# jmhb0/view_neti

Hardware: AMD Instinct MI355X
Metric: TI train steps/sec (SD-1.5 512^2 bs=4 per GPU) (higher is better)
Workload: dtype f16; 1 GPU; learnable_mode 0, sd15 shapes, 512x512 fp16, bs=4/GPU, grad_accum 1, full train step (VAE+16xCLIP+UNet fwd/bwd+AdamW); global_batch=4, parallelism=dp1, rccl_ranks=1, hipgraph=True

## Files before the change

include/vneti.h:

```cpp
#ifndef VNETI_H
#define VNETI_H
#include <stddef.h>
#include <stdint.h>

#ifdef __cplusplus
extern "C" {
#endif

#define VNETI_ABI_VERSION 1

int vneti_version(void);
int vneti_precision(void);
int vneti_last_error(char* buf, size_t n);

typedef struct vneti_gemm_desc {
  const void* A;
  const void* B;
  void* C;
  long long lda, ldb, ldc;
  int M, N, K;
  int batch;
  long long strideA, strideB, strideC;
  const float* bias;
  const void* rowadd;
  long long ld_rowadd;
  int rows_per_group;
  const void* resid;
  long long ldr;
  float alpha;
  int act;
  int out_f32;
  int conv_mode;
  int Hi, Wi, Ci, Ho, Wo, stride, pad_t, pad_l, ups;
  long long ldx;
  int tile_hint;
  void* workspace;
  long long workspace_bytes;
  int split_k;
  const void* gate_src;
  long long ld_gate;
  int gate_act;
  void* C2;
  long long ldc2;
  int act2;
  void* gn_sums;
  int gn_hw, gn_cpg, gn_groups, gn_slots;
  int geglu;
  int conv_korder;
} vneti_gemm_desc;

int vneti_gemm_f16(const vneti_gemm_desc* d, void* stream);
int vneti_gemm_select_tile(int M, int N, int batch);
int vneti_gemm_select_split(int M, int N, int K, int batch, int tile_hint, long long workspace_bytes);

int vneti_im2col3x3_small(const void* x, int x_is_f32, long long sb, long long sc, long long sy,
                          long long sx, void* out, int Bn, int C, int Hi, int Wi, int Ho, int Wo,
                          int stride, int pad_t, int pad_l, void* stream);

int vneti_conv3x3_in(const void* x, int x_is_f32, long long sb, long long sc, long long sy, long long sx,
                     const void* w_packed, const float* bias, void* out, long long ldo, int Bn, int C, int H, int W,
                     int Co, void* gn_sums, int gn_groups, int gn_slots, void* stream);

int vneti_transpose_f16(const void* in, long long ld_in, long long stride_in, void* out,
                        long long ld_out, long long stride_out, int rows, int cols, int batch,
                        void* stream);
#define VNETI_TRANSPOSE_MAX 4
typedef struct vneti_transpose_desc {
  const void* inp;
  long long ld_in, stride_in;
  void* out;
  long long ld_out, stride_out;
  int rows, cols, batch, _pad;
} vneti_transpose_desc;
int vneti_transpose_f16_multi(const vneti_transpose_desc* descs, int n, void* stream);

long long vneti_groupnorm_ws_floats(int Bn, int HW, int C, int G);
int vneti_groupnorm_fwd(const void* x, long long ldx, void* y, long long ldy, const float* gamma,
                        const float* beta, float* mean, float* rstd, float* ws, int Bn, int HW,
                        int C, int G, float eps, int silu, void* stream);
int vneti_groupnorm_fwd_sums(const void* x, long long ldx, void* y, long long ldy, const float* gamma,
                             const float* beta, const void* sums, int slots, float* mean, float* rstd,
                             int Bn, int HW, int C, int G, float eps, int silu, void* stream);
int vneti_groupnorm_fwd_2l(const void* x, long long ldx, void* y, long long ldy, const float* gamma,
                           const float* beta, void* sums, int slots, float* mean, float* rstd, int Bn, int HW,
                           int C, int G, float eps, int silu, void* stream);
int vneti_groupnorm_bwd_2l(const void* dy, long long lddy, const void* x, long long ldx, const float* gamma,
                           const float* beta, const float* mean, const float* rstd, void* dx, long long lddx,
                           const void* dx_accum, long long ldacc, void* sums, int slots, float* ws, int Bn,
                           int HW, int C, int G, int silu, void* stream);
int vneti_groupnorm_bwd(const void* dy, long long lddy, const void* x, long long ldx,
                        const float* gamma, const float* beta, const float* mean,
                        const float* rstd, void* dx, long long lddx, const void* dx_accum,
                        long long ldacc, float* ws, int Bn, int HW, int C, int G, int silu,
                        void* stream);

int vneti_layernorm_fwd(const void* x, int x_is_f32, long long ldx, void* y, long long ldy,
                        const float* gamma, const float* beta, float* mean, float* rstd, int rows,
                        int C, float eps, void* stream);
int vneti_layernorm_bwd(const void* dy, int dy_is_f32, long long lddy, const void* x,
                        int x_is_f32, long long ldx, const float* gamma, const float* mean,
                        const float* rstd, void* dx, int dx_is_f32, long long lddx,
                        const void* dx_accum, long long ldacc, void* dx_f16_copy, long long ldcopy,
                        int rows, int C, void* stream);

int vneti_attn_fwd(const void* Q, long long ldq, const void* K, long long ldk, const void* V,
                   long long ldv, void* O, long long ldo, float* lse, int Bn, int H, int Nq,
// ... 156 lines not shown
```

view_neti_amd/csrc/gemm8.hip:

```cpp
#include <type_traits>

#include "common.h"
#include "gemm_args.h"

namespace {

constexpr int BM = 256, NT = 512;
constexpr int HALF_BYTES = 128 * 128;
constexpr int GN_IMG = 5;

#define VN_WAIT_VM(n) asm volatile("s_waitcnt vmcnt(" #n ")" ::: "memory")
#define VN_WAIT_LGKM0() asm volatile("s_waitcnt lgkmcnt(0)" ::: "memory")

template <int BN, int EPI, bool CONV, bool HALO = false>
__global__ __launch_bounds__(NT) void gemm8_kernel(GemmArgs g) {
  static_assert(BN == 256 || BN == 128, "tile width");
  static_assert(!HALO || (BN == 128 && CONV), "the halo-patch loop exists for the 256x128 convolution tile");
  constexpr int PATCH_STRIDE = 41 * 1024;
  constexpr bool H42 = HALO && BN == 128;
  constexpr int NJB = BN / 128;
  constexpr int HB_BYTES = (BN / 2) * 128;
  constexpr int HB_DMA = BN / 128;
  constexpr int NBUF = BN == 256 ? 2 : 3;
  constexpr int BUF_BYTES = 2 * HALF_BYTES + 2 * HB_BYTES;
  constexpr int CS_LD = BN + 8;
  constexpr int CS_BYTES = BM * CS_LD * 2;
  constexpr int LOOP_BYTES = HALO ? 2 * PATCH_STRIDE + 3 * 2 * HB_BYTES : NBUF * BUF_BYTES;
  constexpr int LDS_BYTES = CS_BYTES > LOOP_BYTES ? CS_BYTES : LOOP_BYTES;
  constexpr int GN_NG = BN / 4 + 2;
  const half_t* const e_gate = EPI == 2 ? g.gate_src : nullptr;
  half_t* const e_C2 = EPI == 2 ? g.C2 : nullptr;
  const int e_geglu = EPI == 2 ? g.geglu : 0;
  const int e_act = EPI == 2 ? g.act : 0;
  float* const e_gn_sums = EPI >= 1 ? g.gn_sums : nullptr;
  const half_t* const e_rowadd = EPI >= 1 ? g.rowadd : nullptr;
  const int e_conv = CONV ? g.conv_mode : 0;
  constexpr int GN_BYTES = EPI == 0 ? 0 : GN_IMG * GN_NG * 4 * 8;
  __shared__ __attribute__((aligned(16))) char smem[LDS_BYTES + GN_BYTES];

  const int tid = threadIdx.x;
  const int lane = tid & 63;
  const int wave = __builtin_amdgcn_readfirstlane(tid >> 6);
  const int wr = wave >> 2, wc = wave & 3;

  int nblk = g.tiles_m * g.tiles_n;
  int bid = blockIdx.x;
  {
    int q = nblk >> 3, r = nblk & 7, xcd = bid & 7, idx = bid >> 3;
    bid = (xcd < r ? xcd * (q + 1) : r * (q + 1) + (xcd - r) * q) + idx;
  }
  const int tile_m = bid / g.tiles_n;
  const int tile_n = bid - tile_m * g.tiles_n;
  const int m0 = tile_m * BM;
  const int n0 = tile_n * BN;
  const int bz = blockIdx.y;
  const int kz = blockIdx.z;
  int hb = 0, hty = 0, htx = 0, row0 = m0;
  if constexpr (HALO) {
    const int tpr = g.Wo >> 4, tpi = (g.Ho >> 4) * tpr;
    hb = tile_m / tpi;
    const int rem = tile_m - hb * tpi;
    hty = rem / tpr;
    htx = rem - hty * tpr;
    row0 = (hb * g.Ho + hty * 16) * g.Wo + htx * 16;
  }
  auto rowmem = [&](const int r) { return HALO ? row0 + (r >> 4) * g.Wo + (r & 15) : m0 + r; };

  const half_t* Ab = g.A + (long long)bz * g.strideA;
  const half_t* Bb = g.B + (long long)bz * g.strideB;
  const __amdgpu_buffer_rsrc_t rsA = vn_make_rsrc(Ab, g.a_bytes);
  const __amdgpu_buffer_rsrc_t rsB = vn_make_rsrc(Bb, g.b_bytes);

  const int lrow = tid >> 3;
  const int gchunk = (tid & 7) ^ ((lrow >> 1) & 7);
  const float rcp_hw = CONV ? 1.0f / (float)(g.Ho * g.Wo) : 0.f, rcp_wo = CONV ? 1.0f / (float)g.Wo : 0.f;
  int a_base[4];
  uint32_t a_mask[4];
#pragma unroll
  for (int r = 0; r < (HALO ? 0 : 4); ++r) {
    const int m = m0 + (r >> 1) * 128 + (r & 1) * 64 + lrow;
// ... 100 lines not shown
#pragma unroll
    for (int j = 0; j < 2; ++j)
      dma16(rsA, dst + j * 8192, nxt[j]);
  };
  auto issueB = [&](const int h, const int buf) {
    char* dst = smem + buf * BUF_BYTES + 2 * HALF_BYTES + h * HB_BYTES + wave * 1024;
    if constexpr (BN == 256) {
#pragma unroll
      for (int j = 0; j < 2; ++j) dma16(rsB, dst + j * 8192, nxt[j]);
    } else {
      dma16(rsB, dst, nxt[2 + h]);
    }
  };

  const int frow = lane & 15;
  const int fq = lane >> 4;
  const int fkey = (frow >> 1) & 7;
  int rdA[2], rdB[2];
#pragma unroll
  for (int s = 0; s < 2; ++s) {
    const int ch = ((s * 4 + fq) ^ fkey) << 4;
    rdA[s] = (wr * 64 + frow) * 128 + ch;
    rdB[s] = 2 * HALF_BYTES + (wc * (16 * NJB) + frow) * 128 + ch;
  }
  half8 af[4][2], bf0[NJB][2], bf1[NJB][2];
  auto readA = [&](const int h) {
#pragma unroll
    for (int i = 0; i < 4; ++i)
#pragma unroll
      for (int s = 0; s < 2; ++s)
        af[i][s] = as_half8(*reinterpret_cast<const u32x4*>(smem + rdA[s] + h * HALF_BYTES + i * 2048));
  };
  auto readB0 = [&](const int flip) {
#pragma unroll
    for (int jb = 0; jb < NJB; ++jb)
#pragma unroll
      for (int s = 0; s < 2; ++s)
        bf0[jb][s] = as_half8(*reinterpret_cast<const u32x4*>(smem + (rdB[s] ^ flip) + jb * 2048));
  };
  auto readB1 = [&]() {
#pragma unroll
    for (int jb = 0; jb < NJB; ++jb)
#pragma unroll
      for (int s = 0; s < 2; ++s)
        bf1[jb][s] = as_half8(*reinterpret_cast<const u32x4*>(smem + rdB[s] + HB_BYTES + jb * 2048));
  };

  const int wr4 = wave >> 1, wc2 = wave & 1;
  auto acc_row = [&](const int h, const int i) { return H42 ? wr4 * 64 + i * 16 + frow : h * 128 + wr * 64 + i * 16 + frow; };
  auto acc_col = [&](const int h, const int j, const int jb) {
    return H42 ? wc2 * 64 + (2 * h + j) * 16 + 4 * fq : j * (BN / 2) + wc * (16 * NJB) + jb * 16 + 4 * fq;
  };
  f32x4 bv[H42 ? 2 : 1][2][NJB];
  {
    const __amdgpu_buffer_rsrc_t rsBias = vn_make_rsrc(g.bias, g.bias ? (uint32_t)g.N * 4u : 0u);
#pragma unroll
    for (int h = 0; h < (H42 ? 2 : 1); ++h)
#pragma unroll
      for (int j = 0; j < 2; ++j)
#pragma unroll
        for (int jb = 0; jb < NJB; ++jb)
          bv[h][j][jb] = __builtin_bit_cast(f32x4, vn_buf_load16(rsBias, (uint32_t)(n0 + acc_col(h, j, jb)) * 4u));
  }
  f32x4 acc[2][2][4][NJB];
#pragma unroll
  for (int h = 0; h < 2; ++h)
#pragma unroll
    for (int j = 0; j < 2; ++j)
#pragma unroll
      for (int i = 0; i < 4; ++i)
#pragma unroll
        for (int jb = 0; jb < NJB; ++jb) acc[h][j][i][jb] = f32x4{0.f, 0.f, 0.f, 0.f};

#define VN_MMA(H, J, BF, PREP)                                                                                 \
  do {                                                                                                         \
    VN_WAIT_LGKM0();                                                                                           \
    __builtin_amdgcn_s_setprio(1);                                                                             \
    PREP;                                                                                                      \
    _Pragma("unroll") for (int s = 0; s < 2; ++s) _Pragma("unroll") for (int i = 0; i < 4; ++i)                \
        _Pragma("unroll") for (int jb = 0; jb < NJB; ++jb) acc[H][J][i][jb] =                                  \
            VN_MFMA_16x16x32(BF[jb][s], af[i][s], acc[H][J][i][jb], 0, 0, 0);                                  \
    __builtin_amdgcn_s_setprio(0);                                                                             \
  } while (0)
#define VN_PHASE_SYNC()                    \
  do {                                     \
    VN_WAIT_VM(10);                        \
    __builtin_amdgcn_s_barrier();          \
    __builtin_amdgcn_sched_barrier(0);     \
  } while (0)
#define VN_PHASE_END()                     \
  do {                                     \
    __builtin_amdgcn_s_barrier();          \
    __builtin_amdgcn_sched_barrier(0);     \
  } while (0)

#define VN_MMA2(H, PREP)                                                                                       \
  do {                                                                                                         \
    VN_WAIT_LGKM0();                                                                                           \
    __builtin_amdgcn_s_setprio(1);                                                                             \
    PREP;                                                                                                      \
    _Pragma("unroll") for (int s = 0; s < 2; ++s) _Pragma("unroll") for (int i = 0; i < 4; ++i) {              \
      acc[H][0][i][0] = VN_MFMA_16x16x32(bf0[0][s], af[i][s], acc[H][0][i][0], 0, 0, 0);                       \
      acc[H][1][i][0] = VN_MFMA_16x16x32(bf1[0][s], af[i][s], acc[H][1][i][0], 0, 0, 0);                       \
    }                                                                                                          \
    __builtin_amdgcn_s_setprio(0);                                                                             \
  } while (0)
#define VN_SYNC(n)                         \
  do {                                     \
    VN_WAIT_VM(n);                         \
    __builtin_amdgcn_s_barrier();          \
    __builtin_amdgcn_sched_barrier(0);     \
  } while (0)
  if constexpr (HALO) {
    constexpr int BRING = 2 * PATCH_STRIDE;
    auto patch_key = [](const int px) { return (int)((0x270745032ull >> (4 * (px >> 1))) & 7); };
    constexpr int PROW = 18 * 128;
    const int c_begin = kt_begin / 9, c_end = kt_end / 9;
    uint32_t pa_off[6];
#pragma unroll
    for (int j = 0; j < 6; ++j) {
      const int q = (j * 8 + wave) * 64 + lane, p = q >> 3, cs = q & 7;
      const int py = (p * 3641) >> 16;
      const int px = p - py * 18;
      const int iy = hty * 16 + py - 1, ix = htx * 16 + px - 1;
      const bool ok = p < 324 && (unsigned)iy < (unsigned)g.Hi && (unsigned)ix < (unsigned)g.Wi;
      pa_off[j] = ok ? (uint32_t)(((hb * g.Hi + iy) * g.Wi + ix) * g.ldx2 + ((cs ^ patch_key(px)) << 4)) : VN_OOB;
    }
    const int np_wave = wave == 0 ? 6 : 5;
    auto issueP = [&](const int j, const int chunk) {
      dma16(rsA, smem + (chunk & 1) * PATCH_STRIDE + (j * 8 + wave) * 1024, pa_off[j] + (uint32_t)chunk * 128u);
    };
    auto tap_dy = [&](const int tap) { const int dy = (tap * 11) >> 5; return e_conv == 2 ? 2 - dy : dy; };
    auto tap_dx = [&](const int tap) { const int dx = tap - 3 * ((tap * 11) >> 5); return e_conv == 2 ? 2 - dx : dx; };
    {
      constexpr int BBUF = 2 * HB_BYTES;
      auto issueBt = [&](const int kt, const int buf) {
        const uint32_t soff = (uint32_t)(kt_begin + kt) * 128u, dead = kt < T ? 0u : VN_OOB;
        char* dst = smem + BRING + buf * BBUF + wave * 1024;
        dma16(rsB, dst, (b_base[0] + soff) | dead);
        dma16(rsB, dst + HB_BYTES, (b_base[2] + soff) | dead);
      };
      int lb[3];
#pragma unroll
      for (int dx = 0; dx < 3; ++dx) lb[dx] = (wr4 * 4) * PROW + (frow + dx) * 128 + ((fq ^ patch_key(frow + dx)) << 4);
      const int rb0 = (wc2 * 64 + frow) * 128 + ((fq ^ fkey) << 4);
      half8 bfh[4][2];
      auto readAh = [&](const int half, const int ab) {
#pragma unroll
        for (int i = 2 * half; i < 2 * half + 2; ++i) {
          af[i][0] = as_half8(*reinterpret_cast<const u32x4*>(smem + ab + i * PROW));
          af[i][1] = as_half8(*reinterpret_cast<const u32x4*>(smem + (ab ^ 64) + i * PROW));
        }
      };
#define VN_MMA4(HALF, PREP)                                                                                    \
  do {                                                                                                         \
    VN_WAIT_LGKM0();                                                                                           \
    __builtin_amdgcn_s_setprio(1);                                                                             \
    PREP;                                                                                                      \
    _Pragma("unroll") for (int s = 0; s < 2; ++s) _Pragma("unroll") for (int i = 2 * HALF; i < 2 * HALF + 2; ++i) \
        _Pragma("unroll") for (int cb = 0; cb < 4; ++cb) {                                                     \
      acc[cb >> 1][cb & 1][i][0] =                                                                             \
          VN_MFMA_16x16x32(bfh[cb][s], af[i][s], acc[cb >> 1][cb & 1][i][0], 0, 0, 0);                         \
    }                                                                                                          \
    __builtin_amdgcn_s_setprio(0);                                                                             \
  } while (0)
      int abt[9];
#pragma unroll
      for (int k = 0; k < 9; ++k) {
        const int tp = e_conv == 2 ? 8 - k : k, dy = tp / 3, dx = tp - 3 * dy;
        abt[k] = (dx == 0 ? lb[0] : (dx == 1 ? lb[1] : lb[2])) + dy * PROW + (c_begin & 1) * PATCH_STRIDE;
      }
      uint32_t bo0 = b_base[0] + (uint32_t)(kt_begin + 2) * 128u, bo1 = b_base[2] + (uint32_t)(kt_begin + 2) * 128u;
      uint32_t pp[6];
#pragma unroll
      for (int j = 0; j < 6; ++j) pp[j] = pa_off[j] + (uint32_t)(c_begin + 1) * 128u;
      const bool w0 = wave == 0;
      char* const bring = smem + BRING + wave * 1024;
      auto readBh = [&](const int slot) {
        const char* b = smem + BRING + slot * BBUF;
#pragma unroll
        for (int cb = 0; cb < 4; ++cb) {
          bfh[cb][0] = as_half8(*reinterpret_cast<const u32x4*>(b + cb * 2048 + rb0));
          bfh[cb][1] = as_half8(*reinterpret_cast<const u32x4*>(b + cb * 2048 + (rb0 ^ 64)));
        }
      };
#pragma unroll
      for (int j = 0; j < 6; ++j)
// ... 112 lines not shown
      cur ^= 1;
#pragma unroll
      for (int s = 0; s < 2; ++s) {
        rdA[s] ^= BUF_BYTES;
        rdB[s] ^= BUF_BYTES;
      }
    }
  } else {
#pragma unroll
    for (int t0 = 0; t0 < 2; ++t0) {
      prepA(0);
      prepB(0);
      prepB(1);
      issueA(0, t0);
      issueB(0, t0);
      issueB(1, t0);
      prepA(1);
      issueA(1, t0);
    }
    prepA(0);
    prepB(0);
    prepB(1);
    VN_WAIT_VM(8);
    __builtin_amdgcn_s_barrier();
    __builtin_amdgcn_sched_barrier(0);
    if (wr == 1) __builtin_amdgcn_s_barrier();
    __builtin_amdgcn_sched_barrier(0);
    int stg = 2;
    for (int t = 0; t < T; ++t) {
      readB0(0);
      readB1();
      readA(0);
      issueA(0, stg);
      issueB(0, stg);
      issueB(1, stg);
      VN_SYNC(10);
      VN_MMA2(0, prepA(1));
      VN_PHASE_END();
      readA(1);
      issueA(1, stg);
      VN_SYNC(8);
      VN_MMA2(1, (prepA(0), prepB(0), prepB(1)));
      VN_PHASE_END();
      stg = stg == 2 ? 0 : stg + 1;
#pragma unroll
      for (int s = 0; s < 2; ++s) {
        rdA[s] = rdA[s] >= 2 * BUF_BYTES ? rdA[s] - 2 * BUF_BYTES : rdA[s] + BUF_BYTES;
        rdB[s] = rdB[s] >= 2 * BUF_BYTES ? rdB[s] - 2 * BUF_BYTES : rdB[s] + BUF_BYTES;
      }
    }
#undef VN_MMA2
#undef VN_SYNC
  }
  if (wr == 0) __builtin_amdgcn_s_barrier();
  asm volatile("s_waitcnt vmcnt(0) lgkmcnt(0)" ::: "memory");
  __syncthreads();
#undef VN_MMA
#undef VN_PHASE_SYNC
#undef VN_PHASE_END

  if (g.ksplit > 1) {
    float* ws = g.ws + ((long long)(kz * g.batch + bz) * g.M) * g.N;
    const __amdgpu_buffer_rsrc_t rsW = vn_make_rsrc(ws, 0x7fffffffu);
#pragma unroll
    for (int h = 0; h < 2; ++h)
#pragma unroll
      for (int j = 0; j < 2; ++j)
#pragma unroll
        for (int i = 0; i < 4; ++i)
#pragma unroll
          for (int jb = 0; jb < NJB; ++jb) {
            const int m = rowmem(acc_row(h, i));
            const int n = n0 + acc_col(h, j, jb);
            if (m < g.M && n < g.N) {
              float* p = ws + (long long)m * g.N + n;
              if (n + 4 <= g.N && (g.N & 3) == 0) {
                vn_st16_wt(rsW, (uint32_t)(((long long)m * g.N + n) * 4), acc[h][j][i][jb]);
              } else {
                for (int e = 0; e < 4 && n + e < g.N; ++e) p[e] = acc[h][j][i][jb][e];
              }
            }
          }
    return;
  }

  if (e_gn_sums && !(HALO && g.gn_hw == g.Ho * g.Wo)) {
    vn_u64* gacc = reinterpret_cast<vn_u64*>(smem + LDS_BYTES);
    for (int i = tid; i < GN_IMG * GN_NG * 4; i += NT) gacc[i] = 0;
  }
  {
    const int nsw = ((frow >> 3) & 1) << 2;
#pragma unroll
    for (int h = 0; h < 2; ++h)
#pragma unroll
      for (int i = 0; i < 4; ++i)
#pragma unroll
        for (int j = 0; j < 2; ++j)
#pragma unroll
          for (int jb = 0; jb < NJB; ++jb) {
            const int ml = acc_row(h, i);
            const int nl = acc_col(h, j, jb) ^ nsw;
            half4 o;
#pragma unroll
            for (int e = 0; e < 4; ++e)
              o[e] = (half_t)apply_act(acc[h][j][i][jb][e] * g.alpha + bv[H42 ? h : 0][j][jb][e], e_act);
            *reinterpret_cast<half4*>(smem + ((size_t)ml * CS_LD + nl) * 2) = o;
          }
  }
  __syncthreads();

  half_t* Cb = reinterpret_cast<half_t*>(g.C) + (long long)bz * g.strideC;
  const __amdgpu_buffer_rsrc_t rsC = vn_make_rsrc(Cb, 0x7fffffffu);
  const __amdgpu_buffer_rsrc_t rsC2 = vn_make_rsrc(e_C2, e_C2 ? 0x7fffffffu : 0u);
  const half_t* Rb = reinterpret_cast<const half_t*>(g.resid);
  if (Rb) Rb += (long long)bz * g.strideC;
  constexpr int CPR = BN / 8;
  constexpr int U = EPI == 2 ? 2 : (EPI == 1 ? 4 : (BN == 256 ? 8 : 4));
  static_assert(NT % CPR == 0 && CPR <= 32 && (BM * CPR) % NT == 0, "a thread keeps one 8-column chunk over all its rows");
  vn_u64* gacc = reinterpret_cast<vn_u64*>(smem + LDS_BYTES);
  const bool gn = e_gn_sums != nullptr;
  const float rcp_gnhw = gn ? 1.0f / (float)g.gn_hw : 0.f, rcp_rpg = e_rowadd ? 1.0f / (float)g.rows_per_group : 0.f;
  const int gn_img0 = gn ? row0 / g.gn_hw : 0, gn_g0t = gn ? n0 / g.gn_cpg : 0;
  const int c = (tid % CPR) * 8;
  const int n = n0 + c;
  const int gn_glo = gn ? n / g.gn_cpg : 0;
  const int gn_split = gn ? (gn_glo + 1) * g.gn_cpg - n : 8;
  int gn_img = -1;
  float s_lo = 0.f, q_lo = 0.f, s_hi = 0.f, q_hi = 0.f;
  auto gn_flush = [&]() {
    const int iref = __builtin_amdgcn_readfirstlane(gn_img);
    const bool uni = __all(gn_img == iref) && iref >= 0;
    if (uni) {
#pragma unroll
      for (int off = 32; off >= CPR; off >>= 1) {
        s_lo += __shfl_xor(s_lo, off);
        q_lo += __shfl_xor(q_lo, off);
        s_hi += __shfl_xor(s_hi, off);
        q_hi += __shfl_xor(q_hi, off);
      }
    }
    if (gn_img >= 0 && (!uni || lane < CPR)) {
      vn_u64* a = gacc + ((gn_img - gn_img0) * GN_NG + (gn_glo - gn_g0t)) * 4;
      vn_fx_add2(a, s_lo, q_lo);
      if (gn_split < 8) vn_fx_add2(a + 4, s_hi, q_hi);
    }
    s_lo = q_lo = s_hi = q_hi = 0.f;
  };
  const bool full_chunk = n + 8 <= g.N;
  const bool swap_halves = ((tid / CPR) >> 3) & 1;
  const __amdgpu_buffer_rsrc_t rsR = vn_make_rsrc(Rb, Rb ? 0x7fffffffu : 0u);
  const __amdgpu_buffer_rsrc_t rsRA = vn_make_rsrc(e_rowadd, e_rowadd ? 0x7fffffffu : 0u);
  const __amdgpu_buffer_rsrc_t rsG = vn_make_rsrc(e_gate, e_gate ? 0x7fffffffu : 0u);
  const int r_first = tid / CPR;
  constexpr int RPP = NT / CPR;
  const bool gn_one = HALO && gn && g.gn_hw == g.Ho * g.Wo;
  const bool ra_one = HALO && EPI >= 1 && e_rowadd && g.rows_per_group == g.Ho * g.Wo;
  half8 av_tile = half8{0, 0, 0, 0, 0, 0, 0, 0};
  if (ra_one) av_tile = as_half8(vn_buf_load16(rsRA, full_chunk ? (uint32_t)(((long long)hb * g.ld_rowadd + n) * 2) : VN_OOB));
  if (gn_one) gn_img = hb;
  for (int it0 = 0; it0 < BM / RPP; it0 += U) {
    half8 cv[U], rv[U], av[U], gv[U], gv2[U];
#pragma unroll
    for (int u = 0; u < U; ++u) {
      const int r = r_first + RPP * (it0 + u);
      const int m = rowmem(r);
      const bool ok = m < g.M && full_chunk;
      u32x4 t = *reinterpret_cast<const u32x4*>(smem + ((size_t)r * CS_LD + c) * 2);
      if (swap_halves) t = u32x4{t[2], t[3], t[0], t[1]};
      cv[u] = as_half8(t);
      if (Rb) rv[u] = as_half8(vn_buf_load16(rsR, ok ? (uint32_t)(((long long)m * g.ldr + n) * 2) : VN_OOB));
      if (EPI >= 1) {
        if (ra_one) {
          av[u] = av_tile;
        } else if (e_rowadd) {
          int grp = (int)((float)m * rcp_rpg);
          const int rem = m - grp * g.rows_per_group;
          grp += rem >= g.rows_per_group ? 1 : (rem < 0 ? -1 : 0);
          av[u] = as_half8(vn_buf_load16(rsRA, ok ? (uint32_t)(((long long)grp * g.ld_rowadd + n) * 2) : VN_OOB));
        }
      }
      if (EPI == 2 && e_gate) {
        const long long go = (long long)m * g.ld_gate + (e_geglu == 2 ? 2 * n : n);
        gv[u] = as_half8(vn_buf_load16_once(rsG, ok ? (uint32_t)(go * 2) : VN_OOB));
        gv2[u] = as_half8(vn_buf_load16_once(rsG, (ok && e_geglu == 2) ? (uint32_t)(go * 2 + 16) : VN_OOB));
// ... 10 lines not shown
          img = (int)((float)m * rcp_gnhw);
          const int rem = m - img * g.gn_hw;
          img += rem >= g.gn_hw ? 1 : (rem < 0 ? -1 : 0);
        }
        if (__any(img != gn_img)) {
          gn_flush();
          gn_img = img;
        }
      }
      if (!valid) continue;
      half8 v = cv[u];
      if (full_chunk) {
        if (EPI >= 1 && e_rowadd) {
          v = vn_add8(v, av[u]);
        }
        if (Rb) {
          v = vn_add8(v, rv[u]);
        }
        if (e_geglu == 2) {
#pragma unroll
          for (int c2 = 0; c2 < 2; ++c2) {
            const half8 pre = c2 == 0 ? gv[u] : gv2[u];
            half8 o;
#pragma unroll
            for (int e = 0; e < 4; ++e) {
              const float d = (float)v[4 * c2 + e], hh = (float)pre[e], gg = (float)pre[4 + e];
              float cdf, xpdf;
              vn_gelu_parts(gg, cdf, xpdf);
              o[e] = (half_t)(d * gg * cdf);
              o[4 + e] = (half_t)(d * hh * (cdf + xpdf));
            }
            vn_st16_wt(rsC, (uint32_t)(((long long)m * g.ldc + 2 * n + 8 * c2) * 2), o);
          }
          continue;
        }
        if (e_gate) {
#pragma unroll
          for (int e = 0; e < 8; ++e) v[e] = (half_t)((float)v[e] * act_grad((float)gv[u][e], g.gate_act));
        }
        if (e_geglu == 1 || (e_C2 && e_geglu == 0)) vn_st16_wt_saved(rsC, (uint32_t)(((long long)m * g.ldc + n) * 2), v);
        else vn_st16_wt(rsC, (uint32_t)(((long long)m * g.ldc + n) * 2), v);
        if (e_geglu == 1) {
          half4 o2;
#pragma unroll
          for (int e = 0; e < 4; ++e) o2[e] = (half_t)((float)v[e] * vn_gelu_erf((float)v[4 + e]));
          *reinterpret_cast<half4*>(e_C2 + (long long)m * g.ldc2 + (n >> 1)) = o2;
        }
        if (gn) {
          {
            const half2v one2 = {(half_t)1.f, (half_t)1.f};
#pragma unroll
            for (int e = 0; e < 8; e += 2) {
              const half2v p2 = {v[e], v[e + 1]};
              if (e < gn_split) {
                s_lo = VN_FDOT2(p2, one2, s_lo);
                q_lo = VN_FDOT2(p2, p2, q_lo);
              } else {
                s_hi = VN_FDOT2(p2, one2, s_hi);
                q_hi = VN_FDOT2(p2, p2, q_hi);
              }
            }
          }
        }
        if (e_C2 && e_geglu == 0) {
          half8 o2;
#pragma unroll
          for (int e = 0; e < 8; ++e) o2[e] = (half_t)apply_act((float)v[e], g.act2);
          vn_st16_wt(rsC2, (uint32_t)(((long long)m * g.ldc2 + n) * 2), o2);
        }
      } else {
        const half_t* radd = e_rowadd ? e_rowadd + (long long)(m / g.rows_per_group) * g.ld_rowadd + n : nullptr;
        for (int e = 0; e < 8 && n + e < g.N; ++e) {
          float x = (float)v[e];
          if (radd) x = (float)(half_t)(x + (float)radd[e]);
          if (Rb) x = (float)(half_t)(x + (float)Rb[(long long)m * g.ldr + n + e]);
          if (e_gate) x = (float)(half_t)(x * act_grad((float)e_gate[(long long)m * g.ld_gate + n + e], g.gate_act));
          Cb[(long long)m * g.ldc + n + e] = (half_t)x;
          if (e_C2) e_C2[(long long)m * g.ldc2 + n + e] = (half_t)apply_act((float)(half_t)x, g.act2);
          if (gn) {
            const float xs = (float)(half_t)x;
            if (e < gn_split) {
              s_lo += xs;
              q_lo += xs * xs;
            } else {
              s_hi += xs;
              q_hi += xs * xs;
            }
          }
        }
      }
    }
  }
  if (gn_one) {
    float v4[4] = {s_lo, q_lo, s_hi, q_hi};
#pragma unroll
    for (int k = 0; k < 4; ++k) {
      v4[k] += __shfl_xor(v4[k], 32);
      v4[k] += __shfl_xor(v4[k], 16);
    }
    static_assert(CPR == 16 || !HALO, "the halo tile is 128 columns wide");
    float* tab = reinterpret_cast<float*>(smem + LDS_BYTES);
    if (lane < 16) *reinterpret_cast<f32x4*>(tab + (wave * 16 + lane) * 4) = f32x4{v4[0], v4[1], v4[2], v4[3]};
    __syncthreads();
    if (tid < 32) {
      const int col = tid >> 1, half = tid & 1;
      float sv = 0.f, qv = 0.f;
#pragma unroll
      for (int w8 = 0; w8 < 8; ++w8) {
        sv += tab[(w8 * 16 + col) * 4 + 2 * half];
        qv += tab[(w8 * 16 + col) * 4 + 2 * half + 1];
      }
      const int nc = n0 + col * 8;
      const int glo = nc / g.gn_cpg;
      const int split = (glo + 1) * g.gn_cpg - nc;
      if (nc < g.N && (half == 0 || split < 8)) {
        const int slot = tile_m % g.gn_slots;
        vn_u64* dst = reinterpret_cast<vn_u64*>(e_gn_sums) + (((long long)hb * g.gn_slots + slot) * g.gn_G + glo + half) * 4;
        vn_fx_add2(dst, sv, qv);
      }
    }
  } else if (gn) {
    gn_flush();
    __syncthreads();
    const int slot = tile_m % g.gn_slots;
    for (int i = tid; i < GN_IMG * GN_NG; i += NT) {
      const vn_u64* src = gacc + 4 * i;
      if ((src[0] | src[1] | src[2] | src[3]) == 0) continue;
      const int img = gn_img0 + i / GN_NG, grp = gn_g0t + i % GN_NG;
      vn_u64* dst = reinterpret_cast<vn_u64*>(e_gn_sums) + (((long long)img * g.gn_slots + slot) * g.gn_G + grp) * 4;
#pragma unroll
      for (int w = 0; w < 4; ++w) atomicAdd(dst + w, src[w]);
    }
  }
}

inline int epilogue_level8(const GemmArgs& g) {
  if (g.gate_src || g.C2 || g.geglu || g.act) return 2;
  return (g.gn_sums || g.rowadd) ? 1 : 0;
}

}

int vneti_launch_gemm8(void* gemm_args, int bn, int halo, hipStream_t st) {
  GemmArgs& g = *reinterpret_cast<GemmArgs*>(gemm_args);
  if (g.out_f32 || (g.conv_mode && (g.ups || (g.conv_mode == 2 && g.stride == 2))) ||
      (g.M >= (1 << 24) && (g.conv_mode || g.rowadd || g.gn_sums)))
    return VNETI_EUNSUP;
  if (halo && (bn != 128 || g.conv_mode < 1 || g.conv_mode > 2 || g.stride != 1 || g.pad_t != 1 || g.pad_l != 1 || g.Hi != g.Ho ||
               g.Wi != g.Wo || (g.Ho & 15) || (g.Wo & 15) || (g.Ci & 63) || g.K != 9 * g.Ci || !g.korder ||
               g.batch != 1 || g.M != (g.M / (g.Ho * g.Wo)) * g.Ho * g.Wo))
    return VNETI_EUNSUP;
  if (halo && g.ksplit > 1) {
    const int nchunk = g.Ci / 64, cps = cdiv(nchunk, g.ksplit);
    g.kt_per_split = 9 * cps;
    g.ksplit = cdiv(nchunk, cps);
  }
  g.tiles_m = cdiv(g.M, BM);
  g.tiles_n = cdiv(g.N, bn);
  const dim3 grid(g.tiles_m * g.tiles_n, g.batch, g.ksplit), block(NT);
  const int epi = epilogue_level8(g);
#define VN_GO(E, C)                                                                        \
  do {                                                                                     \
    if (bn == 256) hipLaunchKernelGGL((gemm8_kernel<256, E, C>), grid, block, 0, st, g);   \
    else hipLaunchKernelGGL((gemm8_kernel<128, E, C>), grid, block, 0, st, g);             \
  } while (0)
#define VN_GO_HALO(E) hipLaunchKernelGGL((gemm8_kernel<128, E, true, true>), grid, block, 0, st, g)
  if (halo) {
    if (epi == 2) VN_GO_HALO(2); else if (epi == 1) VN_GO_HALO(1); else VN_GO_HALO(0);
  } else if (g.conv_mode) {
    if (epi == 2) VN_GO(2, true); else if (epi == 1) VN_GO(1, true); else VN_GO(0, true);
  } else {
    if (epi == 2) VN_GO(2, false); else if (epi == 1) VN_GO(1, false); else VN_GO(0, false);
  }
#undef VN_GO
#undef VN_GO_HALO
  return vneti_check_launch("gemm8_kernel");
}
```

view_neti_amd/lib.py:

```python
from __future__ import annotations

import ctypes as C
import keyword
import os
import re

_HERE = os.path.dirname(os.path.abspath(__file__))
HEADER_PATH = os.path.join(os.path.dirname(_HERE), "include", "vneti.h")

_PRECISIONS = {"fp16": ("libvneti_hip.so", 0), "bf16": ("libvneti_hip_bf16.so", 1)}
_precision = os.environ.get("VNETI_PRECISION", "fp16")
if _precision not in _PRECISIONS:
    raise RuntimeError(f"VNETI_PRECISION={_precision!r}: expected one of {sorted(_PRECISIONS)}")

_lib = None


def so_path(precision: str = None) -> str:
    return os.environ.get("VNETI_LIB_PATH") or os.path.join(_HERE, "csrc", _PRECISIONS[precision or _precision][0])


SO_PATH = so_path()


# ... 27 lines not shown
        return _SCALARS[base]
    if stars == 1 and base == "char":
        return C.c_char_p
    if stars == 1 and base in structs:
        return C.POINTER(structs[base])
    if stars and (base in _SCALARS or base in ("void", "char")):
        return C.c_void_p
    raise ValueError(f"vneti.h {where}: no ctypes rule for the type {ctype.strip()!r}")


def _declarator(decl: str, where: str):
    m = re.fullmatch(r"(.*[\s*])(\w+)", decl.strip(), re.S)
    if not m:
        raise ValueError(f"vneti.h {where}: cannot read the declaration {' '.join(decl.split())!r}")
    return m.group(1), m.group(2)


def parse_header(text: str):
    blank = lambda m: "\n" * m.group().count("\n")
    text = re.sub(r"/\*.*?\*/|//[^\n]*", blank, text, flags=re.S)
    text = re.sub(r'^[ \t]*#.*$|extern\s+"C"\s*\{|^\}[ \t]*$', "", text, flags=re.M)
    at = lambda src, pos: f"line {src.count(chr(10), 0, pos) + 1}"
    structs, protos = {}, {}
    typedef = r"typedef\s+struct\s+\w*\s*\{(.*?)\}\s*(\w+)\s*;"
    for m in re.finditer(typedef, text, flags=re.S):
        fields = []
        for d in re.finditer(r"[^;\s][^;]*", m.group(1)):
            where = at(text, m.start(1) + d.start())
            first, *more = d.group().split(",")
            ctype, name = _declarator(first, where)
            for n in [name] + [x.strip() for x in more]:
                if not n.isidentifier() or keyword.iskeyword(n):
                    raise ValueError(f"vneti.h {where}: cannot bind the field {n!r}")
                fields.append((n, _ctype(ctype, structs, where)))
        structs[m.group(2)] = type(m.group(2), (C.Structure,), {"_fields_": fields})
    rest = re.sub(typedef, blank, text, flags=re.S)
    for m in re.finditer(r"[^;\s][^;]*", rest):
        p = re.fullmatch(r"(int|long long)\s+(vneti_\w+)\s*\((.*)\)\s*", m.group(), re.S)
        if not p:
            raise ValueError(f"vneti.h {at(rest, m.start())}: cannot read {' '.join(m.group().split())!r} as a prototype")
        argtypes = []
        for x in re.finditer(r"[^,\s][^,]*", "" if p.group(3).strip() == "void" else p.group(3)):
            where = at(rest, m.start() + p.start(3) + x.start())
            argtypes.append(_ctype(_declarator(x.group(), where)[0], structs, where))
        protos[p.group(2)] = (_SCALARS[p.group(1)], argtypes)
    return structs, protos


with open(HEADER_PATH) as _f:
    _STRUCTS, _PROTOS = parse_header(_f.read())
GemmDesc, TransposeDesc = _STRUCTS["vneti_gemm_desc"], _STRUCTS["vneti_transpose_desc"]
SIGNATURES = {n[len("vneti_"):]: argtypes for n, (_, argtypes) in _PROTOS.items()}
VALUE_FUNCS = frozenset({
    "version", "precision", "last_error", "gemm_select_tile", "gemm_select_split", "img_resample_ksize",
    "groupnorm_ws_floats", "lpips_ws_floats", "mapper_num_params", "mapper_save_floats", "mapper_rowgrad_floats",
    "mapper_legacy_input_params"})
_stray = ({n[len("vneti_"):] for n, (res, _) in _PROTOS.items() if res is C.c_longlong} - VALUE_FUNCS) | (VALUE_FUNCS - set(SIGNATURES))
if _stray:
    raise RuntimeError(f"lib.VALUE_FUNCS is out of step with include/vneti.h: {sorted(_stray)}")


def declared_symbols() -> list[str]:
    src = open(HEADER_PATH).read()
    src = re.sub(r"/\*.*?\*/", "", src, flags=re.S)
    return sorted(set(re.findall(r"\b(vneti_[a-z0-9_]+)\s*\(", src)))


def load():
    global _lib
    if _lib is not None:
        return _lib
    if not os.path.exists(SO_PATH):
        raise RuntimeError(
            f"{os.path.basename(SO_PATH)} not found at {SO_PATH}: build it with "
            "`python view_neti_amd/csrc/build.py` (hipcc, gfx950). There is no fallback path.")
    lib = C.CDLL(SO_PATH)
    for name, (restype, argtypes) in _PROTOS.items():
        fn = getattr(lib, name, None)
        if fn is None:
            raise RuntimeError(f"{SO_PATH} does not export {name}, which include/vneti.h declares: rebuild it")
        fn.restype, fn.argtypes = restype, argtypes
    if lib.vneti_precision() != _PRECISIONS[_precision][1]:
        raise RuntimeError(f"{SO_PATH} computes in precision {lib.vneti_precision()}, the process asked for {_precision}")
    _lib = lib
    return lib


def last_error() -> str:
    lib = load()
    buf = C.create_string_buffer(512)
    lib.vneti_last_error(buf, 512)
    return buf.value.decode(errors="replace")


def check(rc: int, what: str = ""):
    if rc != 0:
        raise RuntimeError(f"vneti call failed ({what}) rc={rc}: {last_error()}")


def call(name: str, *args):
    check(getattr(load(), "vneti_" + name)(*args), name)


def query(name: str, *args) -> int:
    if name not in VALUE_FUNCS:
        raise KeyError(f"vneti_{name} returns a status: use call()")
    return int(getattr(load(), "vneti_" + name)(*args))
# ... 1 lines not shown
```

view_neti_amd/ops.py:

```python
from __future__ import annotations

import ctypes as C

import torch

from . import lib as _l

ACT_NONE, ACT_SILU, ACT_QUICK_GELU, ACT_GELU = 0, 1, 2, 3


def stream() -> int:
    return torch.cuda.current_stream().cuda_stream


def _p(t):
    return None if t is None else t.data_ptr()


def _ld(t):
    if t is None:
        return 0
    assert t.stride(-1) == 1, "last dim must be contiguous"
    return t.stride(-2) if t.dim() >= 2 else t.shape[-1]

# ... 337 lines not shown
def mapper_legacy_input_fwd(params_in, timesteps, w_pe, enc_out, nl, Bn, enc_dim, pe_dim, slot=None, slot_stride=0):
    _l.call("mapper_legacy_input_fwd", _p(params_in), _p(slot), slot_stride, _p(timesteps), _p(w_pe), _p(enc_out), nl, Bn,
            enc_dim, pe_dim, stream())


def mapper_legacy_input_fwd_slots(params_in, slots, slot_stride, timesteps, w_pe, enc_out, nl, Bn, enc_dim, pe_dim):
    _l.call("mapper_legacy_input_fwd_slots", _p(params_in), _p(slots), slot_stride, _p(timesteps), _p(w_pe), _p(enc_out),
            nl, Bn, enc_dim, pe_dim, stream())


def mapper_legacy_input_bwd(timesteps, w_pe, denc, grads_in, accumulate, nl, Bn, enc_dim, pe_dim, slot=None, slot_stride=0):
    _l.call("mapper_legacy_input_bwd", _p(timesteps), _p(w_pe), _p(denc), _p(grads_in), _p(slot), slot_stride,
            1 if accumulate else 0, nl, Bn, enc_dim, pe_dim, stream())


def text_embed(tok_emb, pos_emb, ids, pos_obj, word_obj, pos_view, word_view, X, nl, Bn, L, D):
    _l.call("text_embed", _p(tok_emb), _p(pos_emb), _p(ids), _p(pos_obj), _p(word_obj), _p(pos_view), _p(word_view),
            _p(X), nl, Bn, L, D, stream())


def text_final_fwd(last, gamma, beta, eps, pos_obj, byp_obj, alpha_obj, pos_view, byp_view, alpha_view, ctx_k, ctx_v,
                   nl, Bn, L, D, unconstrained_obj=False, unconstrained_view=False, norm_terms=None):
    _l.call("text_final_fwd", _p(last), _p(gamma), _p(beta), eps, _p(pos_obj), _p(byp_obj), alpha_obj,
            1 if unconstrained_obj else 0, _p(pos_view), _p(byp_view), alpha_view, 1 if unconstrained_view else 0,
            _p(norm_terms), _p(ctx_k), _p(ctx_v), nl, Bn, L, D, stream())


def text_final_bwd(last, gamma, eps, pos_obj, byp_obj, alpha_obj, dbyp_obj, pos_view, byp_view, alpha_view, dbyp_view,
                   dctx_k, dctx_v, dX, nl, Bn, L, D, unconstrained_obj=False, unconstrained_view=False,
                   norm_terms=None):
    _l.call("text_final_bwd", _p(last), _p(gamma), eps, _p(pos_obj), _p(byp_obj), alpha_obj,
            1 if unconstrained_obj else 0, _p(dbyp_obj), _p(pos_view), _p(byp_view), alpha_view,
            1 if unconstrained_view else 0, _p(dbyp_view), _p(norm_terms), _p(dctx_k), _p(dctx_v), _p(dX), nl, Bn, L,
            D, stream())


def cast_f32_f16(x, y):
    _l.call("cast_f32_f16", _p(x), _p(y), x.numel(), stream())


def mapper_inputs(timesteps, view_params, data, nl, Bn):
    nv = 0 if view_params is None else view_params.shape[1]
    _l.call("mapper_inputs", _p(timesteps), _p(view_params), nv, _p(data), nl, Bn, stream())


def gemm_select_split(M, N, K, batch, tile_hint, workspace_bytes):
    return _l.query("gemm_select_split", M, N, K, batch, tile_hint, workspace_bytes)


def gemm_select_tile(M, N, batch=1):
    return _l.query("gemm_select_tile", M, N, batch)


def lpips_prep(x, out, Bn, H, W):
    assert x.dtype == torch.float32 and x.shape == (Bn, 3, H, W)
    assert out.is_contiguous() and out.numel() >= Bn * H * W * 64
    _l.call("lpips_prep", _p(x), *x.stride(), _p(out), Bn, H, W, stream())


def relu_(x):
    assert x.is_contiguous()
    _l.call("relu_f16", _p(x), x.numel(), stream())


def relu_maxpool2x2(x, out, Bn, H, W, Cc):
    assert x.is_contiguous() and out.is_contiguous() and x.numel() >= Bn * H * W * Cc
    assert out.numel() >= Bn * (H // 2) * (W // 2) * Cc
    _l.call("relu_maxpool2x2_f16", _p(x), _p(out), Bn, H, W, Cc, stream())


def lpips_ws_floats(P, Cc, HW):
    n = _l.query("lpips_ws_floats", P, Cc, HW)
    if n < 0:
        raise RuntimeError(f"lpips_distance: unsupported shape P={P} C={Cc} HW={HW}")
    return n


def lpips_distance(feat, n_img, pairs, w, Cc, HW, ws, out, accumulate=False):
    P = pairs.shape[0]
    assert pairs.dtype == torch.int32 and pairs.is_contiguous() and pairs.shape == (P, 2)
    assert feat.is_contiguous() and feat.numel() >= n_img * HW * Cc and w.dtype == torch.float32 and w.numel() == Cc
    assert out.dtype == torch.float32 and out.numel() >= P and ws.dtype == torch.float32
    _l.call("lpips_distance", _p(feat), n_img, _p(pairs), P, _p(w), Cc, HW, _p(ws), ws.numel(), _p(out),
            1 if accumulate else 0, stream())


def img_resample_ksize(in_size, out_size, filt):
    return _l.query("img_resample_ksize", in_size, out_size, filt)


def img_resample_coeffs(in_size, out_size, filt, bounds, kk):
    _l.call("img_resample_coeffs", in_size, out_size, filt, _p(bounds), _p(kk), stream())


def img_resample_pass(inp, in_w, out, out_h, out_w, bounds, kk, ksize, horizontal):
    _l.call("img_resample_pass", _p(inp), in_w, _p(out), out_h, out_w, _p(bounds), _p(kk), ksize, 1 if horizontal else 0,
            stream())


def img_crop(inp, in_w, top, left, out, h, w, flip=False):
    _l.call("img_crop", _p(inp), in_w, top, left, _p(out), h, w, 1 if flip else 0, stream())


def img_enhance(img, h, w, mode, alpha, scratch8):
    _l.call("img_enhance", _p(img), h, w, mode, float(alpha), _p(scratch8), stream())

# ... 20 lines not shown
```

Measured before the change: 38.71 steps/s.

## Add 256-wide halo-patch convolution tile with wave-occupancy heuristic

Adds a 256x256 variant of the halo-patch implicit-GEMM convolution kernel. It has its own double-buffered B pipeline, a per-tap schedule, bias loading deferred until after the main loop, and a split GroupNorm partial-sum reduction through LDS. A heuristic picks it when N is a multiple of 256 and the estimated number of block waves favours wider tiles. The aim is more reuse of each loaded input patch across output channels and fewer passes over the activations. In exchange it uses more LDS and registers per block and gives fewer blocks per launch. An environment variable and API can force or disable the path.

After: 38.82 steps/s (median of 6 runs). No clear change (+0.3%).

```diff
diff --git a/include/vneti.h b/include/vneti.h
--- a/include/vneti.h
+++ b/include/vneti.h
@@ -52,6 +52,8 @@
 int vneti_gemm_f16(const vneti_gemm_desc* d, void* stream);
 int vneti_gemm_select_tile(int M, int N, int batch);
 int vneti_gemm_select_split(int M, int N, int K, int batch, int tile_hint, long long workspace_bytes);
+int vneti_gemm_halo_wide_set(int mode);
+int vneti_gemm_halo_wide_count(void);
 
 int vneti_im2col3x3_small(const void* x, int x_is_f32, long long sb, long long sc, long long sy,
                           long long sx, void* out, int Bn, int C, int Hi, int Wi, int Ho, int Wo,
diff --git a/view_neti_amd/csrc/gemm8.hip b/view_neti_amd/csrc/gemm8.hip
--- a/view_neti_amd/csrc/gemm8.hip
+++ b/view_neti_amd/csrc/gemm8.hip
@@ -1,3 +1,5 @@
+#include <atomic>
+#include <cstdlib>
 #include <type_traits>
 
 #include "common.h"
@@ -15,7 +17,7 @@
 template <int BN, int EPI, bool CONV, bool HALO = false>
 __global__ __launch_bounds__(NT) void gemm8_kernel(GemmArgs g) {
   static_assert(BN == 256 || BN == 128, "tile width");
-  static_assert(!HALO || (BN == 128 && CONV), "the halo-patch loop exists for the 256x128 convolution tile");
+  static_assert(!HALO || CONV, "the halo-patch loops are convolution tiles");
   constexpr int PATCH_STRIDE = 41 * 1024;
   constexpr bool H42 = HALO && BN == 128;
   constexpr int NJB = BN / 128;
@@ -25,7 +27,8 @@
   constexpr int BUF_BYTES = 2 * HALF_BYTES + 2 * HB_BYTES;
   constexpr int CS_LD = BN + 8;
   constexpr int CS_BYTES = BM * CS_LD * 2;
-  constexpr int LOOP_BYTES = HALO ? 2 * PATCH_STRIDE + 3 * 2 * HB_BYTES : NBUF * BUF_BYTES;
+  constexpr bool H44 = HALO && BN == 256;
+  constexpr int LOOP_BYTES = HALO ? 2 * PATCH_STRIDE + (H44 ? 2 : 3) * 2 * HB_BYTES : NBUF * BUF_BYTES;
   constexpr int LDS_BYTES = CS_BYTES > LOOP_BYTES ? CS_BYTES : LOOP_BYTES;
   constexpr int GN_NG = BN / 4 + 2;
   const half_t* const e_gate = EPI == 2 ? g.gate_src : nullptr;
@@ -232,7 +235,7 @@
     return H42 ? wc2 * 64 + (2 * h + j) * 16 + 4 * fq : j * (BN / 2) + wc * (16 * NJB) + jb * 16 + 4 * fq;
   };
   f32x4 bv[H42 ? 2 : 1][2][NJB];
-  {
+  auto load_bias = [&]() {
     const __amdgpu_buffer_rsrc_t rsBias = vn_make_rsrc(g.bias, g.bias ? (uint32_t)g.N * 4u : 0u);
 #pragma unroll
     for (int h = 0; h < (H42 ? 2 : 1); ++h)
@@ -241,7 +244,8 @@
 #pragma unroll
         for (int jb = 0; jb < NJB; ++jb)
           bv[h][j][jb] = __builtin_bit_cast(f32x4, vn_buf_load16(rsBias, (uint32_t)(n0 + acc_col(h, j, jb)) * 4u));
-  }
+  };
+  if constexpr (!H44) load_bias();
   f32x4 acc[2][2][4][NJB];
 #pragma unroll
   for (int h = 0; h < 2; ++h)
@@ -312,7 +316,137 @@
     };
     auto tap_dy = [&](const int tap) { const int dy = (tap * 11) >> 5; return e_conv == 2 ? 2 - dy : dy; };
     auto tap_dx = [&](const int tap) { const int dx = tap - 3 * ((tap * 11) >> 5); return e_conv == 2 ? 2 - dx : dx; };
-    {
+    if constexpr (H44) {
+      constexpr int BBUF = 2 * HB_BYTES;
+      int lb[3];
+#pragma unroll
+      for (int dx = 0; dx < 3; ++dx) lb[dx] = (wr * 4) * PROW + (frow + dx) * 128 + ((fq ^ patch_key(frow + dx)) << 4);
+      const int rowstep = e_conv == 2 ? -PROW : PROW;
+      int ar[3];
+#pragma unroll
+      for (int d = 0; d < 3; ++d) ar[d] = (e_conv == 2 ? lb[2 - d] + 2 * PROW : lb[d]) + (c_begin & 1) * PATCH_STRIDE;
+      int rbs[2];
+      rbs[0] = BRING + (wc * 32 + frow) * 128 + ((fq ^ fkey) << 4);
+      rbs[1] = rbs[0] + BBUF;
+      int bsl[2] = {BRING + wave * 1024, BRING + BBUF + wave * 1024};
+      uint32_t bo = b_base[0] + (uint32_t)(kt_begin + 2) * 128u;
+      const uint32_t bstep = (uint32_t)g.ldb * 128u;
+      uint32_t pp[6];
+#pragma unroll
+      for (int j = 0; j < 6; ++j) pp[j] = pa_off[j] + (uint32_t)(c_begin + 1) * 128u;
+      const bool w0 = wave == 0;
+      auto readAw = [&](const int h, const int ab0, const int ab1) {
+#pragma unroll
+        for (int i = 0; i < 4; ++i) {
+          af[i][0] = as_half8(*reinterpret_cast<const u32x4*>(smem + ab0 + (h * 8 + i) * PROW));
+          af[i][1] = as_half8(*reinterpret_cast<const u32x4*>(smem + ab1 + (h * 8 + i) * PROW));
+        }
+      };
+      auto readB0w = [&](const int rb) {
+#pragma unroll
+        for (int jb = 0; jb < 2; ++jb) {
+          bf0[jb][0] = as_half8(*reinterpret_cast<const u32x4*>(smem + rb + jb * 2048));
+          bf0[jb][1] = as_half8(*reinterpret_cast<const u32x4*>(smem + (rb ^ 64) + jb * 2048));
+        }
+      };
+      auto readB1w = [&](const int rb) {
+#pragma unroll
+        for (int jb = 0; jb < 2; ++jb) {
+          bf1[jb][0] = as_half8(*reinterpret_cast<const u32x4*>(smem + rb + HB_BYTES + jb * 2048));
+          bf1[jb][1] = as_half8(*reinterpret_cast<const u32x4*>(smem + (rb ^ 64) + HB_BYTES + jb * 2048));
+        }
+      };
+#pragma unroll
+      for (int j = 0; j < 6; ++j)
+        if (j < np_wave) issueP(j, c_begin);
+#pragma unroll
+      for (int kt = 0; kt < 2; ++kt) {
+        const uint32_t soff = (uint32_t)(kt_begin + kt) * 128u, dead = kt < T ? 0u : VN_OOB;
+#pragma unroll
+        for (int r = 0; r < 4; ++r) dma16(rsB, smem + bsl[kt] + r * 8192, (b_base[0] + r * bstep + soff) | dead);
+      }
+      VN_WAIT_VM(6);
+      __builtin_amdgcn_s_barrier();
+      __builtin_amdgcn_sched_barrier(0);
+      readB0w(rbs[0]);
+      VN_WAIT_LGKM0();
+      __builtin_amdgcn_sched_barrier(0);
+      if (wr == 1) __builtin_amdgcn_s_barrier();
+      __builtin_amdgcn_sched_barrier(0);
+      auto ktile = [&](auto tap_c, const bool last_chunk, const int pslot, const int astep) {
+        constexpr int tap = decltype(tap_c)::value;
+        constexpr int par = tap & 1, td = tap % 3;
+        const uint32_t dead = (last_chunk && tap >= 7) ? VN_OOB : 0u;
+        readAw(0, ar[td], ar[td] ^ 64);
+        if constexpr (tap >= 1 && tap <= 6) {
+          if (tap < 6 || w0) {
+            dma16(rsA, smem + pslot + ((tap - 1) * 8) * 1024 + wave * 1024, last_chunk ? VN_OOB : pp[tap - 1]);
+          }
+        }
+        if constexpr (tap >= 2 && tap <= 5) {
+          VN_WAIT_VM(6);
+        } else if constexpr (tap == 1 || tap == 6) {
+          VN_WAIT_VM(5);
+        } else {
+          VN_WAIT_VM(4);
+        }
+        __builtin_amdgcn_s_barrier();
+        __builtin_amdgcn_sched_barrier(0);
+        VN_MMA(0, 0, bf0, (void)0);
+        VN_PHASE_END();
+        readB1w(rbs[par]);
+        dma16(rsB, smem + bsl[par], bo | dead);
+        dma16(rsB, smem + bsl[par] + 8192, (bo + bstep) | dead);
+        __builtin_amdgcn_s_barrier();
+        __builtin_amdgcn_sched_barrier(0);
+        VN_MMA(0, 1, bf1, (void)0);
+        VN_PHASE_END();
+        readAw(1, ar[td], ar[td] ^ 64);
+        if constexpr (tap >= 1 && tap <= 5) {
+          VN_WAIT_VM(5);
+        } else {
+          VN_WAIT_VM(4);
+        }
+        __builtin_amdgcn_s_barrier();
+        __builtin_amdgcn_sched_barrier(0);
+        VN_MMA(1, 0, bf0, (void)0);
+        VN_PHASE_END();
+        readB0w(rbs[par ^ 1]);
+        dma16(rsB, smem + bsl[par] + HB_BYTES, (bo + 2 * bstep) | dead);
+        dma16(rsB, smem + bsl[par] + HB_BYTES + 8192, (bo + 3 * bstep) | dead);
+        __builtin_amdgcn_s_barrier();
+        __builtin_amdgcn_sched_barrier(0);
+        if constexpr (td == 2) {
+          VN_MMA(1, 1, bf1, (bo += 128u, ar[0] += astep, ar[1] += astep, ar[2] += astep));
+        } else {
+          VN_MMA(1, 1, bf1, bo += 128u);
+        }
+        VN_PHASE_END();
+      };
+      for (int c = c_begin; c < c_end; ++c) {
+        const bool last_chunk = c + 1 >= c_end;
+        const int pslot = ((c + 1) & 1) * PATCH_STRIDE;
+        const int nextrow = rowstep, nextchunk = ((c & 1) ? -PATCH_STRIDE : PATCH_STRIDE) - 2 * rowstep;
+        ktile(std::integral_constant<int, 0>{}, last_chunk, pslot, nextrow);
+        ktile(std::integral_constant<int, 1>{}, last_chunk, pslot, nextrow);
+        ktile(std::integral_constant<int, 2>{}, last_chunk, pslot, nextrow);
+        ktile(std::integral_constant<int, 3>{}, last_chunk, pslot, nextrow);
+        ktile(std::integral_constant<int, 4>{}, last_chunk, pslot, nextrow);
+        ktile(std::integral_constant<int, 5>{}, last_chunk, pslot, nextrow);
+        ktile(std::integral_constant<int, 6>{}, last_chunk, pslot, nextrow);
+        ktile(std::integral_constant<int, 7>{}, last_chunk, pslot, nextrow);
+        ktile(std::integral_constant<int, 8>{}, last_chunk, pslot, nextchunk);
+#pragma unroll
+        for (int j = 0; j < 6; ++j) pp[j] += 128u;
+        {
+          const int tr = rbs[0], ts = bsl[0];
+          rbs[0] = rbs[1];
+          rbs[1] = tr;
+          bsl[0] = bsl[1];
+          bsl[1] = ts;
+        }
+      }
+    } else {
       constexpr int BBUF = 2 * HB_BYTES;
       auto issueBt = [&](const int kt, const int buf) {
         const uint32_t soff = (uint32_t)(kt_begin + kt) * 128u, dead = kt < T ? 0u : VN_OOB;
@@ -531,6 +665,7 @@
 #undef VN_MMA2
 #undef VN_SYNC
   }
+  if constexpr (H44) load_bias();
   if (wr == 0) __builtin_amdgcn_s_barrier();
   asm volatile("s_waitcnt vmcnt(0) lgkmcnt(0)" ::: "memory");
   __syncthreads();
@@ -605,10 +740,16 @@
   const int gn_glo = gn ? n / g.gn_cpg : 0;
   const int gn_split = gn ? (gn_glo + 1) * g.gn_cpg - n : 8;
   int gn_img = -1;
-  float s_lo = 0.f, q_lo = 0.f, s_hi = 0.f, q_hi = 0.f;
+  constexpr bool GN2 = H44;
+  float s_lo_[2] = {0.f, 0.f}, q_lo_[2] = {0.f, 0.f}, s_hi_[2] = {0.f, 0.f}, q_hi_[2] = {0.f, 0.f};
+  float &s_lo = s_lo_[0], &q_lo = q_lo_[0], &s_hi = s_hi_[0], &q_hi = q_hi_[0];
   auto gn_flush = [&]() {
     const int iref = __builtin_amdgcn_readfirstlane(gn_img);
     const bool uni = __all(gn_img == iref) && iref >= 0;
+    if constexpr (GN2) {
+      s_lo += s_lo_[1], q_lo += q_lo_[1], s_hi += s_hi_[1], q_hi += q_hi_[1];
+      s_lo_[1] = q_lo_[1] = s_hi_[1] = q_hi_[1] = 0.f;
+    }
     if (uni) {
 #pragma unroll
       for (int off = 32; off >= CPR; off >>= 1) {
@@ -725,12 +866,13 @@
 #pragma unroll
             for (int e = 0; e < 8; e += 2) {
               const half2v p2 = {v[e], v[e + 1]};
+              const int gp = GN2 ? (u & 1) : 0;
               if (e < gn_split) {
-                s_lo = VN_FDOT2(p2, one2, s_lo);
-                q_lo = VN_FDOT2(p2, p2, q_lo);
+                s_lo_[gp] = VN_FDOT2(p2, one2, s_lo_[gp]);
+                q_lo_[gp] = VN_FDOT2(p2, p2, q_lo_[gp]);
               } else {
-                s_hi = VN_FDOT2(p2, one2, s_hi);
-                q_hi = VN_FDOT2(p2, p2, q_hi);
+                s_hi_[gp] = VN_FDOT2(p2, one2, s_hi_[gp]);
+                q_hi_[gp] = VN_FDOT2(p2, p2, q_hi_[gp]);
               }
             }
           }
@@ -764,14 +906,39 @@
       }
     }
   }
-  if (gn_one) {
+  if (GN2 && gn_one) {
+    __syncthreads();
+    float* tab = reinterpret_cast<float*>(smem);
+#pragma unroll
+    for (int b = 0; b < 2; ++b)
+      *reinterpret_cast<f32x4*>(tab + ((r_first + 16 * b) * 32 + (tid & 31)) * 4) = f32x4{s_lo_[b], q_lo_[b], s_hi_[b], q_hi_[b]};
+    __syncthreads();
+    if (tid < 64) {
+      const int col = tid >> 1, half = tid & 1;
+      float sv = 0.f, qv = 0.f;
+#pragma unroll
+      for (int w8 = 0; w8 < 8; ++w8) {
+        const float* t4 = tab + ((4 * w8) * 32 + col) * 4 + 2 * half;
+        sv += (t4[0] + t4[256]) + (t4[128] + t4[384]);
+        qv += (t4[1] + t4[257]) + (t4[129] + t4[385]);
+      }
+      const int nc = n0 + col * 8;
+      const int glo = nc / g.gn_cpg;
+      const int split = (glo + 1) * g.gn_cpg - nc;
+      if (nc < g.N && (half == 0 || split < 8)) {
+        const int slot = tile_m % g.gn_slots;
+        vn_u64* dst = reinterpret_cast<vn_u64*>(e_gn_sums) + (((long long)hb * g.gn_slots + slot) * g.gn_G + glo + half) * 4;
+        vn_fx_add2(dst, sv, qv);
+      }
+    }
+  } else if (gn_one) {
     float v4[4] = {s_lo, q_lo, s_hi, q_hi};
 #pragma unroll
     for (int k = 0; k < 4; ++k) {
       v4[k] += __shfl_xor(v4[k], 32);
       v4[k] += __shfl_xor(v4[k], 16);
     }
-    static_assert(CPR == 16 || !HALO, "the halo tile is 128 columns wide");
+    static_assert(CPR == 16 || !HALO || GN2, "this fold is the 128-wide halo tile's");
     float* tab = reinterpret_cast<float*>(smem + LDS_BYTES);
     if (lane < 16) *reinterpret_cast<f32x4*>(tab + (wave * 16 + lane) * 4) = f32x4{v4[0], v4[1], v4[2], v4[3]};
     __syncthreads();
@@ -812,6 +979,25 @@
   return (g.gn_sums || g.rowadd) ? 1 : 0;
 }
 
+std::atomic<int> g_halo_wide_mode{[] {
+  const char* e = getenv("VNETI_HALO_WIDE");
+  return (e && e[0] >= '0' && e[0] <= '2' && e[1] == 0) ? e[0] - '0' : 1;
+}()};
+std::atomic<int> g_halo_wide_count{0};
+
+inline bool halo_wide(const GemmArgs& g) {
+  const int mode = g_halo_wide_mode.load(std::memory_order_relaxed);
+  if (mode == 0 || (g.N & 255)) return false;
+  if (g.gn_sums && g.gn_hw != g.Ho * g.Wo) return false;
+  const long long wide_blocks = (long long)cdiv(g.M, BM) * (g.N / 256) * g.ksplit;
+  return mode == 2 || 9 * ((wide_blocks + 255) / 256) < 5 * ((2 * wide_blocks + 255) / 256);
+}
+
+}
+
+extern "C" int vneti_gemm_halo_wide_count(void) { return g_halo_wide_count.load(std::memory_order_relaxed); }
+extern "C" int vneti_gemm_halo_wide_set(int mode) {
+  return (mode >= 0 && mode <= 2) ? g_halo_wide_mode.exchange(mode) : g_halo_wide_mode.load();
 }
 
 int vneti_launch_gemm8(void* gemm_args, int bn, int halo, hipStream_t st) {
@@ -828,6 +1014,10 @@
     g.kt_per_split = 9 * cps;
     g.ksplit = cdiv(nchunk, cps);
   }
+  if (halo && halo_wide(g)) {
+    bn = 256;
+    g_halo_wide_count.fetch_add(1, std::memory_order_relaxed);
+  }
   g.tiles_m = cdiv(g.M, BM);
   g.tiles_n = cdiv(g.N, bn);
   const dim3 grid(g.tiles_m * g.tiles_n, g.batch, g.ksplit), block(NT);
@@ -837,7 +1027,11 @@
     if (bn == 256) hipLaunchKernelGGL((gemm8_kernel<256, E, C>), grid, block, 0, st, g);   \
     else hipLaunchKernelGGL((gemm8_kernel<128, E, C>), grid, block, 0, st, g);             \
   } while (0)
-#define VN_GO_HALO(E) hipLaunchKernelGGL((gemm8_kernel<128, E, true, true>), grid, block, 0, st, g)
+#define VN_GO_HALO(E)                                                                            \
+  do {                                                                                           \
+    if (bn == 256) hipLaunchKernelGGL((gemm8_kernel<256, E, true, true>), grid, block, 0, st, g); \
+    else hipLaunchKernelGGL((gemm8_kernel<128, E, true, true>), grid, block, 0, st, g);          \
+  } while (0)
   if (halo) {
     if (epi == 2) VN_GO_HALO(2); else if (epi == 1) VN_GO_HALO(1); else VN_GO_HALO(0);
   } else if (g.conv_mode) {
diff --git a/view_neti_amd/lib.py b/view_neti_amd/lib.py
--- a/view_neti_amd/lib.py
+++ b/view_neti_amd/lib.py
@@ -103,7 +103,8 @@
 GemmDesc, TransposeDesc = _STRUCTS["vneti_gemm_desc"], _STRUCTS["vneti_transpose_desc"]
 SIGNATURES = {n[len("vneti_"):]: argtypes for n, (_, argtypes) in _PROTOS.items()}
 VALUE_FUNCS = frozenset({
-    "version", "precision", "last_error", "gemm_select_tile", "gemm_select_split", "img_resample_ksize",
+    "version", "precision", "last_error", "gemm_select_tile", "gemm_select_split", "gemm_halo_wide_count", "gemm_halo_wide_set",
+    "img_resample_ksize",
     "groupnorm_ws_floats", "lpips_ws_floats", "mapper_num_params", "mapper_save_floats", "mapper_rowgrad_floats",
     "mapper_legacy_input_params"})
 _stray = ({n[len("vneti_"):] for n, (res, _) in _PROTOS.items() if res is C.c_longlong} - VALUE_FUNCS) | (VALUE_FUNCS - set(SIGNATURES))
diff --git a/view_neti_amd/ops.py b/view_neti_amd/ops.py
--- a/view_neti_amd/ops.py
+++ b/view_neti_amd/ops.py
@@ -413,6 +413,14 @@
     return _l.query("gemm_select_tile", M, N, batch)
 
 
+def halo_wide(mode=-1):
+    return _l.query("gemm_halo_wide_set", mode)
+
+
+def halo_wide_count():
+    return _l.query("gemm_halo_wide_count")
+
+
 def lpips_prep(x, out, Bn, H, W):
     assert x.dtype == torch.float32 and x.shape == (Bn, 3, H, W)
     assert out.is_contiguous() and out.numel() >= Bn * H * W * 64
```
